# jafarinia/snuffy

Hardware: AMD Instinct MI355X
Metric: slides/sec (higher is better)
Workload: dtype f32; 1 GPU; cfgB: MILNet eval forward, 1 bag/step/rank, N=32768 patches D=768 h=6 Lambda=200 (K=200) depth=1 relu mlp x4; parallelism=bag-parallel x1, bags_resident_per_rank=8, launch=hip graph replay, rccl_ranks=0

## Files before the change

### include/snuffy_hip.h

```cpp
#ifndef SNUFFY_HIP_H
#define SNUFFY_HIP_H

#include <stddef.h>
#include <stdint.h>

#ifdef __cplusplus
extern "C" {
#endif

typedef void* snf_stream_t;

#define SNF_OK 0
#define SNF_EINVAL (-1)
#define SNF_ELAUNCH (-2)
#define SNF_EUNSUPPORTED (-3)
#define SNF_EWORKSPACE (-4)

#define SNF_ACT_RELU 0
#define SNF_ACT_GELU 1
#define SNF_ACT_LEAKYRELU 2
#define SNF_ACT_SELU 3
#define SNF_ACT_NONE 4

#define SNF_DT_F32 0
// ... 58 lines not shown
                     const void* gate_bf16, void* dst_bf16, float* partial, snf_stream_t stream);
int snf_dropout_rows_bf16(void* x, int64_t ldx, int64_t m, int n, float dropout_p, uint64_t seed, uint64_t offset, snf_stream_t stream);
int snf_residual_assemble_dropout_f32(const float* x, int64_t n, int d, const void* add_bf16, const float* add_bias,
                                      const int32_t* slot_map, const float* delta_rows, float dropout_p, uint64_t seed, uint64_t offset,
                                      float* z_out, snf_stream_t stream);
int snf_colsum_fused_dropout(const void* src, int src_dtype, int64_t n, int d, float dropout_p, uint64_t seed, uint64_t offset,
                             void* dst_bf16, float* partial, snf_stream_t stream);
int snf_split3_colsum_f32(const float* x, int64_t ldx, int64_t m, int k, const void* gate_bf16, int64_t ldg, void* out_bf16,
                          int64_t ldo, int64_t plane, float* partial, snf_stream_t stream);
int snf_split_hl_colsum_f32(const float* x, int64_t ldx, int64_t m, int k, const void* gate_hl, int64_t ldg, void* out_hl, int64_t ldo,
                            float* partial, snf_stream_t stream);
int snf_linear_rows_x3_f32(const float* x, int64_t ldx, const float* w, int64_t ldw, const float* bias, int r, int c, int k, void* out,
                           int64_t ldo, int out_dtype, snf_stream_t stream);
int snf_linear_rows_x3_resid_f32(const float* x, int64_t ldx, const float* w, int64_t ldw, const float* bias, const float* resid, int64_t ldr,
                                 int r, int c, int k, float* out, int64_t ldo, float* out2, int64_t ldo2, snf_stream_t stream);
int snf_critic_ln_hl_f32(const float* x, int64_t n, int d, const float* w, const float* b, int c_out, float* scores,
                         const float* gamma, const float* beta, float eps, void* out_hl, void* selector_state,
                         snf_stream_t stream);
int snf_layernorm_rows_split3_f32(const float* x, int64_t n, int d, const int32_t* slot_map, const float* patch_rows,
                                  const float* gamma, const float* beta, float eps, void* out_bf16, snf_stream_t stream);

int snf_bias_act(void* h, int dtype, int64_t n, int f, const float* bias, int act, snf_stream_t stream);

size_t snf_ln_mean_head_workspace_bytes(int d);
int snf_ln_mean_head_f32(const float* z, int64_t n, int d, const void* add_bf16, const float* add_bias,
                         const int32_t* slot_map, const float* delta_rows, float* z_out, const float* gamma,
                         const float* beta, float eps, const float* w_head, const float* b_head, int c_out,
                         float* logits, float* pooled, void* workspace, size_t workspace_bytes, snf_stream_t stream);
int snf_ln_mean_head_deferred_f32(const float* z, int64_t n, int d, const float* slabs, const int32_t* tile_map, int tiles_n,
                                  const void* add_bf16, const float* add_bias, const int32_t* slot_map, const float* delta_rows,
                                  float* z_out, const float* gamma, const float* beta, float eps, const float* w_head,
                                  const float* b_head, int c_out, float* logits, float* pooled, void* workspace,
                                  size_t workspace_bytes, snf_stream_t stream);

size_t snf_sparse_attn_fwd_workspace_bytes(int64_t n, int k, int h, int dk, int mfma);
int snf_sparse_attn_fwd_f32(const float* q, const float* kp, const float* v, int64_t n, int k, int h, int dk,
                            float scale, float* out, float* attn, float* lse, void* workspace,
                            size_t workspace_bytes, snf_stream_t stream);
int snf_sparse_attn_fwd_x3u_f32(const float* q, int64_t ldq, const float* kp, const float* v, int64_t ldv, int64_t n, int k, int h, int dk,
                                float scale, float* out, float* attn, float* lse, void* workspace, size_t workspace_bytes,
                                snf_stream_t stream);
int snf_sparse_attn_fwd_mfma(const void* q, int64_t ldq, const void* v, int64_t ldv, int qv_dtype, const void* kp,
                             int kp_dtype, int64_t n, int k, int h, int dk, float scale, float* out, float* attn,
                             float* lse, void* workspace, size_t workspace_bytes, snf_stream_t stream);

int snf_sparse_attn_fwd_mfma_dropout(const void* q, int64_t ldq, const void* v, int64_t ldv, int qv_dtype, const void* kp,
                                     int kp_dtype, int64_t n, int k, int h, int dk, float scale, float* out, float* attn,
                                     float* lse, float dropout_p, uint64_t seed, uint64_t offset, void* workspace,
                                     size_t workspace_bytes, snf_stream_t stream);
int snf_sparse_attn_bwd_mfma_dropout(const void* q, int64_t ldq, const void* v, int64_t ldv, int qv_dtype, const float* kp,
                                     const float* dout, const float* lse, const float* mask, float dropout_p, uint64_t seed,
                                     uint64_t offset, int64_t n, int k, int h, int dk, float scale, float* dq, float* dv,
                                     void* ds, int ds_dtype, snf_stream_t stream);
int snf_dropout_mask_f32(float dropout_p, uint64_t seed, uint64_t offset, int h, int64_t n, int k, float* mask,
                         snf_stream_t stream);

size_t snf_sparse_attn_fwd_x3_workspace_bytes(int64_t n, int k, int h, int dk);
int snf_sparse_attn_fwd_x3(const float* q, int64_t ldq, const float* v, int64_t ldv, const float* kp, int64_t n, int k, int h,
                           int dk, float scale, float* out, float* attn, float* lse, void* workspace, size_t workspace_bytes,
                           snf_stream_t stream);
int snf_sparse_attn_fwd_x3_dropout(const float* q, int64_t ldq, const float* v, int64_t ldv, const float* kp, int64_t n, int k, int h,
                                   int dk, float scale, float dropout_p, uint64_t seed, uint64_t offset, float* out, float* attn,
                                   float* lse, void* workspace, size_t workspace_bytes, snf_stream_t stream);

size_t snf_sparse_attn_fwd_x3_hl_workspace_bytes(int64_t n, int k, int h, int dk);
int snf_sparse_attn_fwd_x3_hl(const void* q_hl, int64_t ldq, const void* v_hl, int64_t ldv, const float* kp, int64_t n, int k, int h,
// ... 150 lines not shown
```

### snuffy_amd/_ffi.py

```python
import ctypes
import os
from ctypes import c_char_p, c_float, c_int, c_int64, c_size_t, c_uint64, c_void_p

_HERE = os.path.dirname(os.path.abspath(__file__))
LIB_PATH = os.environ.get("SNUFFY_HIP_LIB") or os.path.join(_HERE, "lib", "libsnuffy_hip.so")

SNF_OK = 0
SNF_EINVAL = -1
SNF_ELAUNCH = -2
SNF_EUNSUPPORTED = -3
SNF_EWORKSPACE = -4

ACT_CODES = {"relu": 0, "gelu": 1, "leakyrelu": 2, "selu": 3, "none": 4}
DT_F32 = 0
DT_BF16 = 1
DT_BF16_SPLIT3 = 2
DT_BF16_HL = 3
TOPK_MAX_K = 2048

SIGNATURES = {
    "snf_version": (c_char_p, []),
    "snf_last_error": (c_char_p, []),
    "snf_device_cu_count": (c_int, []),
    "snf_critic_f32": (c_int, [c_void_p, c_int64, c_int, c_void_p, c_void_p, c_int, c_void_p, c_void_p, c_void_p,
# ... 15 lines not shown
    "snf_slot_map_i32": (c_int, [c_void_p, c_int, c_int64, c_void_p, c_void_p]),
    "snf_gather_slot_map_f32": (c_int, [c_void_p, c_int64, c_int, c_void_p, c_int, c_void_p, c_void_p, c_void_p, c_void_p]),
    "snf_layernorm_rows_f32": (c_int, [c_void_p, c_int64, c_int, c_void_p, c_void_p, c_void_p, c_void_p, c_float,
                                       c_void_p, c_void_p, c_void_p, c_void_p, c_void_p, c_void_p]),
    "snf_layernorm_bwd_blocks": (c_int, [c_int64]),
    "snf_layernorm_rows_bwd_f32": (c_int, [c_void_p, c_int64, c_int, c_void_p, c_int, c_int64, c_void_p, c_float, c_void_p,
                                           c_void_p, c_void_p, c_void_p, c_void_p]),
    "snf_fold_blocks": (c_int, [c_int]),
    "snf_fold_linear_f32": (c_int, [c_void_p, c_int, c_int, c_void_p, c_void_p, c_void_p, c_void_p, c_int64, c_void_p, c_void_p,
                                    c_void_p]),
    "snf_unfold_linear_f32": (c_int, [c_void_p, c_void_p, c_int, c_int, c_void_p, c_void_p, c_void_p, c_void_p, c_void_p,
                                      c_void_p]),
    "snf_split3_f32": (c_int, [c_void_p, c_int64, c_int64, c_int, c_void_p, c_void_p]),
    "snf_mil_loss_f32": (c_int, [c_void_p, c_int64, c_int, c_void_p, c_void_p, c_void_p, c_void_p, c_void_p, c_void_p, c_void_p, c_void_p]),
    "snf_mil_loss_bwd_f32": (c_int, [c_void_p, c_void_p, c_void_p, c_int64, c_int, c_void_p, c_void_p, c_void_p]),
    "snf_split3_weight_f32": (c_int, [c_void_p, c_int64, c_int64, c_int, c_void_p, c_void_p, c_void_p]),
    "snf_split3_colsum_f32": (c_int, [c_void_p, c_int64, c_int64, c_int, c_void_p, c_int64, c_void_p, c_int64, c_int64, c_void_p, c_void_p]),
    "snf_colsum_blocks": (c_int, [c_int64]),
    "snf_colsum_fused": (c_int, [c_void_p, c_int, c_int64, c_int, c_void_p, c_int64, c_void_p, c_void_p, c_void_p, c_void_p]),
    "snf_layernorm_rows_split3_f32": (c_int, [c_void_p, c_int64, c_int, c_void_p, c_void_p, c_void_p, c_void_p, c_float,
                                              c_void_p, c_void_p]),
    "snf_linear_rows_x3_f32": (c_int, [c_void_p, c_int64, c_void_p, c_int64, c_void_p, c_int, c_int, c_int, c_void_p, c_int64, c_int,
                                       c_void_p]),
    "snf_critic_ln_hl_f32": (c_int, [c_void_p, c_int64, c_int, c_void_p, c_void_p, c_int, c_void_p, c_void_p, c_void_p, c_float,
                                     c_void_p, c_void_p, c_void_p]),
    "snf_bias_act": (c_int, [c_void_p, c_int, c_int64, c_int, c_void_p, c_int, c_void_p]),
    "snf_ln_mean_head_workspace_bytes": (c_size_t, [c_int]),
    "snf_ln_mean_head_f32": (c_int, [c_void_p, c_int64, c_int, c_void_p, c_void_p, c_void_p, c_void_p, c_void_p,
                                     c_void_p, c_void_p, c_float, c_void_p, c_void_p, c_int, c_void_p, c_void_p,
                                     c_void_p, c_size_t, c_void_p]),
    "snf_ln_mean_head_deferred_f32": (c_int, [c_void_p, c_int64, c_int, c_void_p, c_void_p, c_int, c_void_p, c_void_p, c_void_p, c_void_p,
                                              c_void_p, c_void_p, c_void_p, c_float, c_void_p, c_void_p, c_int, c_void_p, c_void_p,
                                              c_void_p, c_size_t, c_void_p]),
    "snf_sparse_attn_fwd_workspace_bytes": (c_size_t, [c_int64, c_int, c_int, c_int, c_int]),
    "snf_sparse_attn_fwd_f32": (c_int, [c_void_p, c_void_p, c_void_p, c_int64, c_int, c_int, c_int, c_float, c_void_p,
                                        c_void_p, c_void_p, c_void_p, c_size_t, c_void_p]),
    "snf_sparse_attn_fwd_x3u_f32": (c_int, [c_void_p, c_int64, c_void_p, c_void_p, c_int64, c_int64, c_int, c_int, c_int, c_float, c_void_p,
                                            c_void_p, c_void_p, c_void_p, c_size_t, c_void_p]),
    "snf_sparse_attn_bwd_workspace_bytes": (c_size_t, [c_int64, c_int, c_int, c_int]),
    "snf_sparse_attn_bwd_f32": (c_int, [c_void_p, c_void_p, c_void_p, c_void_p, c_void_p, c_void_p, c_int64, c_int, c_int,
                                        c_int, c_float, c_void_p, c_void_p, c_void_p, c_void_p, c_size_t, c_void_p]),
    "snf_sparse_attn_bwd_ld_f32": (c_int, [c_void_p, c_int64, c_void_p, c_void_p, c_int64, c_void_p, c_void_p, c_void_p, c_int64, c_int, c_int,
                                           c_int, c_float, c_void_p, c_void_p, c_void_p, c_void_p, c_size_t, c_void_p]),
    "snf_sparse_attn_bwd_dropout_f32": (c_int, [c_void_p, c_int64, c_void_p, c_void_p, c_int64, c_void_p, c_float, c_uint64, c_uint64, c_void_p,
                                                c_int64, c_int, c_int, c_int, c_float, c_void_p, c_void_p, c_void_p, c_void_p, c_size_t, c_void_p]),
    "snf_sparse_attn_bwd_mfma": (c_int, [c_void_p, c_int64, c_void_p, c_int64, c_int, c_void_p, c_void_p, c_void_p, c_void_p,
                                         c_int64, c_int, c_int, c_int, c_float, c_void_p, c_void_p, c_void_p, c_int, c_void_p]),
    "snf_sparse_attn_dkp_f32": (c_int, [c_void_p, c_void_p, c_int64, c_int, c_int, c_int, c_void_p, c_void_p, c_size_t,
                                        c_void_p]),
    "snf_sparse_attn_fwd_mfma": (c_int, [c_void_p, c_int64, c_void_p, c_int64, c_int, c_void_p, c_int, c_int64, c_int, c_int,
                                         c_int, c_float, c_void_p, c_void_p, c_void_p, c_void_p, c_size_t, c_void_p]),
    "snf_sparse_attn_fwd_x3_workspace_bytes": (c_size_t, [c_int64, c_int, c_int, c_int]),
    "snf_sparse_attn_fwd_x3": (c_int, [c_void_p, c_int64, c_void_p, c_int64, c_void_p, c_int64, c_int, c_int, c_int, c_float,
                                       c_void_p, c_void_p, c_void_p, c_void_p, c_size_t, c_void_p]),
    "snf_sparse_attn_fwd_x3_dropout": (c_int, [c_void_p, c_int64, c_void_p, c_int64, c_void_p, c_int64, c_int, c_int, c_int, c_float,
                                               c_float, c_uint64, c_uint64, c_void_p, c_void_p, c_void_p, c_void_p, c_size_t, c_void_p]),
    "snf_sparse_attn_fwd_x3_hl_workspace_bytes": (c_size_t, [c_int64, c_int, c_int, c_int]),
    "snf_sparse_attn_x3_hl_kpfrag_bytes": (c_size_t, [c_int, c_int, c_int]),
    "snf_linear_rows_x3_kpfrag_f32": (c_int, [c_void_p, c_int64, c_void_p, c_int64, c_void_p, c_int, c_int, c_int, c_int, c_float,
                                              c_void_p, c_size_t, c_void_p]),
    "snf_gather_linear_rows_x3_kpfrag_f32": (c_int, [c_void_p, c_int64, c_int64, c_void_p, c_void_p, c_int64, c_void_p, c_int, c_int, c_int,
                                                     c_int, c_float, c_void_p, c_size_t, c_void_p, c_void_p, c_void_p]),
    "snf_sparse_attn_fwd_x3_hl_kpfrag": (c_int, [c_void_p, c_int64, c_void_p, c_int64, c_void_p, c_int64, c_int, c_int, c_int,
                                                 c_void_p, c_void_p, c_void_p, c_void_p, c_size_t, c_void_p]),
    "snf_sparse_attn_fwd_x3_hl": (c_int, [c_void_p, c_int64, c_void_p, c_int64, c_void_p, c_int64, c_int, c_int, c_int, c_float,
                                          c_void_p, c_void_p, c_void_p, c_void_p, c_size_t, c_void_p]),
# ... 133 lines not shown
```

### snuffy_amd/csrc/rowops.hip

```cpp
#include <math.h>

#include "common.h"
#include "philox.h"
#include "selector.h"

namespace {

constexpr int WG = 256;
constexpr int WAVES = WG / 64;

template <int VEC>
struct VecT;
template <>
struct VecT<4> {
    using type = float4;
};
template <>
struct VecT<1> {
    using type = float;
};

template <int VEC, int NV>
struct RowRegs {
    float v[NV * VEC];
// ... 1017 lines not shown
                    hi += bias[col + 2 * t + 1];
                }
                w[t] = pack_bf16x2(apply_act(lo, act), apply_act(hi, act));
            }
            *reinterpret_cast<uint4*>(h + i8) = make_uint4(w[0], w[1], w[2], w[3]);
        }
    } else {
        for (int64_t i = (int64_t)blockIdx.x * blockDim.x + threadIdx.x; i < total; i += (int64_t)gridDim.x * blockDim.x) {
            float v = bf16_bits_to_f32(h[i]) + (bias ? bias[i % f] : 0.f);
            h[i] = f32_to_bf16_bits(apply_act(v, act));
        }
    }
}

template <int VEC, int NV>
__device__ __forceinline__ void add_row_bf16(const unsigned short* __restrict__ row, int d, int lane, float (&r)[NV * VEC]) {
#pragma unroll
    for (int i = 0; i < NV; ++i) {
        int e = (i * 64 + lane) * VEC;
        if (e < d) {
            if constexpr (VEC == 4) {
                uint2 p = *reinterpret_cast<const uint2*>(row + e);
                r[i * 4 + 0] += __uint_as_float(p.x << 16);
                r[i * 4 + 1] += __uint_as_float(p.x & 0xffff0000u);
                r[i * 4 + 2] += __uint_as_float(p.y << 16);
                r[i * 4 + 3] += __uint_as_float(p.y & 0xffff0000u);
            } else {
                r[i] += bf16_bits_to_f32(row[e]);
            }
        }
    }
}

template <int VEC, int NV, bool DEFER = false>
__global__ __launch_bounds__(WG) void ln_colsum_kernel(const float* __restrict__ z, int64_t n, int d, float eps,
                                                       const unsigned short* __restrict__ add_bf16,
                                                       const float* __restrict__ add_bias,
                                                       const int32_t* __restrict__ slot_map,
                                                       const float* __restrict__ delta_rows,
                                                       float* __restrict__ z_out,
                                                       float* __restrict__ partial ,
                                                       const int* __restrict__ vl = nullptr, int vl_bags = 0,
                                                       const float* __restrict__ slabs = nullptr,
                                                       const int32_t* __restrict__ tile_map = nullptr, int tiles_n = 0) {
    const int lane = threadIdx.x & 63;
    const int wave = threadIdx.x >> 6;
    int bid = blockIdx.x, gdim = gridDim.x;
    if (vl) {
        const int* __restrict__ dsc = vl + 4 * vl[4 * vl_bags + bid];
        const int64_t row0 = dsc[1];
        bid -= dsc[0];
        n = dsc[2];
        gdim = dsc[3];
        z += row0 * d;
        if (add_bf16) add_bf16 += row0 * d;
        if (slot_map) slot_map += row0;
        if (z_out) z_out += row0 * d;
    }
    float acc[NV * VEC];
#pragma unroll
    for (int i = 0; i < NV * VEC; ++i) acc[i] = 0.f;
    float bias_r[NV * VEC];
    if (add_bias) load_row<VEC, NV>(add_bias, d, lane, bias_r);
    const float inv_d = 1.0f / (float)d;
    const int64_t rstride = (int64_t)gdim * WAVES;
    float nz[NV * VEC];
    uint2 nb[NV];
    constexpr int NCB = DEFER ? (NV * VEC * 64 + 255) / 256 : 1;
    float ns[DEFER ? NV * VEC : 1];
    int mp_n[NCB], mp_nn[NCB];
    auto lookup = [&](int64_t row, int (&mp)[NCB]) __attribute__((always_inline)) {
        const int trow = __builtin_amdgcn_readfirstlane((int)(row >> 8));
#pragma unroll
        for (int cb = 0; cb < NCB; ++cb) mp[cb] = cb < tiles_n ? tile_map[(int64_t)trow * tiles_n + cb] : 0;
    };
    auto issue = [&](int64_t row) __attribute__((always_inline)) {
        load_row<VEC, NV>(z + row * d, d, lane, nz);
// ... 75 lines not shown
            int sl = slot_map[row];
            if (sl >= 0) {
                float dr[NV * VEC];
                load_row<VEC, NV>(delta_rows + (int64_t)sl * d, d, lane, dr);
#pragma unroll
                for (int i = 0; i < NV * VEC; ++i) r[i] += dr[i];
            }
        }
        if (z_out) store_row_f32<VEC, NV>(z_out + row * d, d, lane, r);
        float s1 = 0.f;
#pragma unroll
        for (int i = 0; i < NV * VEC; ++i) s1 += r[i];
        const float mean = wave_sum(s1) * inv_d;
        float s2 = 0.f;
#pragma unroll
        for (int i = 0; i < NV; ++i) {
#pragma unroll
            for (int t = 0; t < VEC; ++t) {
                int e = (i * 64 + lane) * VEC + t;
                float dv = (e < d) ? (r[i * VEC + t] - mean) : 0.f;
                s2 = fmaf(dv, dv, s2);
            }
        }
        const float rstd = 1.0f / sqrtf(wave_sum(s2) * inv_d + eps);
#pragma unroll
        for (int i = 0; i < NV * VEC; ++i) acc[i] += (r[i] - mean) * rstd;
    }
    extern __shared__ float lds[];
    float* mine = lds + wave * (NV * VEC * 64);
#pragma unroll
    for (int i = 0; i < NV * VEC; ++i) mine[i * 64 + lane] = acc[i];
    __syncthreads();
    if (wave == 0) {
#pragma unroll
        for (int i = 0; i < NV; ++i) {
#pragma unroll
            for (int t = 0; t < VEC; ++t) {
                float s = 0.f;
                for (int w2 = 0; w2 < WAVES; ++w2) s += lds[w2 * (NV * VEC * 64) + (i * VEC + t) * 64 + lane];
                int e = (i * 64 + lane) * VEC + t;
                if (e < d) partial[(int64_t)blockIdx.x * d + e] = s;
            }
        }
    }
}

constexpr int HEAD_NSLICE = 16;
__global__ __launch_bounds__(256) void ln_colreduce_kernel(const float* __restrict__ partial, int nparts, int d,
                                                           float* __restrict__ partial2 ,
                                                           const int* __restrict__ vl = nullptr) {
    __shared__ float red[4][64];
    if (vl) {
        const int* __restrict__ dsc = vl + 4 * blockIdx.z;
        partial += (int64_t)dsc[0] * d;
        nparts = dsc[3];
        partial2 += (int64_t)blockIdx.z * HEAD_NSLICE * d;
    }
    const int c = threadIdx.x & 63, wv = threadIdx.x >> 6;
    const int e = blockIdx.x * 64 + c;
    const int sl = blockIdx.y;
    float s = 0.f;
    if (e < d)
        for (int p = sl + HEAD_NSLICE * wv; p < nparts; p += HEAD_NSLICE * 4) s += partial[(int64_t)p * d + e];
    red[wv][c] = s;
    __syncthreads();
    if (wv == 0 && e < d) partial2[(int64_t)sl * d + e] = ((red[0][c] + red[1][c]) + red[2][c]) + red[3][c];
}

__global__ __launch_bounds__(256) void head_gemv_kernel(const float* __restrict__ partial2, int64_t n, int d,
                                                        const float* __restrict__ gamma, const float* __restrict__ beta,
                                                        const float* __restrict__ w_head, const float* __restrict__ b_head,
                                                        float* __restrict__ pooled_out, float* __restrict__ logits,
                                                        const int* __restrict__ vl = nullptr) {
    __shared__ float red[256];
    if (vl) {
        partial2 += (int64_t)blockIdx.y * HEAD_NSLICE * d;
        n = vl[4 * blockIdx.y + 2];
        logits += (int64_t)blockIdx.y * gridDim.x;
        if (pooled_out) pooled_out += (int64_t)blockIdx.y * d;
    }
// ... 670 lines not shown
                "snf_gather_slot_map_f32: bad shape n=%lld d=%d k=%d (k <= 2048)", (long long)n, d, k);
    const int64_t grid = k + (n + WG - 1) / WG;
    hipLaunchKernelGGL(gather_slot_map_kernel, dim3((unsigned)grid), dim3(WG), 0, snf::as_stream(stream), x, n, d, idx, k, xs,
                       map, reinterpret_cast<__bf16*>(xs_bf16));
    return snf::check_launch("gather_slot_map_kernel");
}

int snf_bias_act(void* h, int dtype, int64_t n, int f, const float* bias, int act, snf_stream_t stream) {
    SNF_REQUIRE(h, "snf_bias_act: null h");
    SNF_REQUIRE(n >= 1 && f >= 1, "snf_bias_act: bad shape");
    SNF_REQUIRE(act >= SNF_ACT_RELU && act <= SNF_ACT_NONE, "snf_bias_act: unknown activation %d", act);
    SNF_REQUIRE(dtype == SNF_DT_F32 || dtype == SNF_DT_BF16, "snf_bias_act: unknown dtype %d", dtype);
    SNF_REQUIRE(aligned16(h) && (!bias || aligned16(bias)), "snf_bias_act: buffers must be 16-byte aligned");
    const int64_t total = n * (int64_t)f;
    const int per = dtype == SNF_DT_F32 ? 4 : 8;
    int64_t want = (total / per + WG - 1) / WG;
    int64_t cap = (int64_t)snf::cu_count() * 8;
    int grid = (int)(want < cap ? (want > 0 ? want : 1) : cap);
    hipStream_t s = snf::as_stream(stream);
    if (dtype == SNF_DT_F32)
        hipLaunchKernelGGL(bias_act_f32_kernel, dim3(grid), dim3(WG), 0, s, reinterpret_cast<float*>(h), n, f, bias, act);
    else
        hipLaunchKernelGGL(bias_act_bf16_kernel, dim3(grid), dim3(WG), 0, s, reinterpret_cast<unsigned short*>(h), n, f,
                           bias, act);
    return snf::check_launch("bias_act_kernel");
}

static int ln_head_parts(int64_t n) {
    int64_t want = (n + WAVES - 1) / WAVES;
    int64_t cap = (int64_t)snf::cu_count() * 4;
    return (int)(want < cap ? (want > 0 ? want : 1) : cap);
}

size_t snf_ln_mean_head_workspace_bytes(int d) {
    if (d < 1) return 0;
    return ((size_t)snf::cu_count() * 4 + HEAD_NSLICE) * (size_t)d * sizeof(float);
}

static int ln_mean_head_impl(const float* z, int64_t n, int d, const float* slabs, const int32_t* tile_map, int tiles_n,
                             const void* add_bf16, const float* add_bias, const int32_t* slot_map, const float* delta_rows,
                             float* z_out, const float* gamma, const float* beta, float eps, const float* w_head,
                             const float* b_head, int c_out, float* logits, float* pooled, void* workspace, size_t workspace_bytes,
                             snf_stream_t stream) {
    SNF_REQUIRE(z && w_head && logits && workspace, "snf_ln_mean_head_f32: null pointer");
    SNF_REQUIRE(!slot_map || delta_rows, "snf_ln_mean_head_f32: slot_map without delta_rows");
    SNF_REQUIRE(n >= 1 && d >= 1 && c_out >= 1, "snf_ln_mean_head_f32: bad shape");
    const int parts = ln_head_parts(n);
    if (workspace_bytes < ((size_t)parts + HEAD_NSLICE) * d * sizeof(float)) {
        snf::set_error("snf_ln_mean_head_f32: workspace %zu < %zu", workspace_bytes,
                       ((size_t)parts + HEAD_NSLICE) * d * sizeof(float));
        return SNF_EWORKSPACE;
    }
    RowCfg cfg;
    const bool al = aligned16(z) && (!add_bf16 || aligned16(add_bf16)) && (!add_bias || aligned16(add_bias)) &&
                    (!delta_rows || aligned16(delta_rows)) && (!z_out || aligned16(z_out));
    SNF_REQUIRE(pick_row_cfg(d, al, &cfg), "snf_ln_mean_head_f32: d=%d too wide (max 2048)", d);
    hipStream_t s = snf::as_stream(stream);
    float* partial = reinterpret_cast<float*>(workspace);
    float* partial2 = partial + (size_t)parts * d;
    if (tile_map) {
        SNF_ROW_DISPATCH(cfg, hipLaunchKernelGGL((ln_colsum_kernel<VEC, NV, true>), dim3(parts), dim3(WG),
                                                  WAVES * NV * VEC * 64 * sizeof(float), s, z, n, d, eps,
                                                  reinterpret_cast<const unsigned short*>(add_bf16), add_bias, slot_map,
                                                  delta_rows, z_out, partial, nullptr, 0, slabs, tile_map, tiles_n));
    } else {
        SNF_ROW_DISPATCH(cfg, hipLaunchKernelGGL((ln_colsum_kernel<VEC, NV>), dim3(parts), dim3(WG),
                                                  WAVES * NV * VEC * 64 * sizeof(float), s, z, n, d, eps,
                                                  reinterpret_cast<const unsigned short*>(add_bf16), add_bias, slot_map,
                                                  delta_rows, z_out, partial));
    }
    int rc = snf::check_launch("ln_colsum_kernel");
    if (rc) return rc;
    hipLaunchKernelGGL(ln_colreduce_kernel, dim3((d + 63) / 64, HEAD_NSLICE), dim3(256), 0, s, partial, parts, d, partial2);
    rc = snf::check_launch("ln_colreduce_kernel");
    if (rc) return rc;
    hipLaunchKernelGGL(head_gemv_kernel, dim3(c_out), dim3(256), 0, s, partial2, n, d, gamma, beta, w_head, b_head, pooled,
                       logits);
    return snf::check_launch("head_gemv_kernel");
}

int snf_ln_mean_head_f32(const float* z, int64_t n, int d, const void* add_bf16, const float* add_bias,
                         const int32_t* slot_map, const float* delta_rows, float* z_out, const float* gamma,
                         const float* beta, float eps, const float* w_head, const float* b_head, int c_out, float* logits,
                         float* pooled, void* workspace, size_t workspace_bytes, snf_stream_t stream) {
    return ln_mean_head_impl(z, n, d, nullptr, nullptr, 0, add_bf16, add_bias, slot_map, delta_rows, z_out, gamma, beta, eps, w_head,
                             b_head, c_out, logits, pooled, workspace, workspace_bytes, stream);
}

int snf_ln_mean_head_deferred_f32(const float* z, int64_t n, int d, const float* slabs, const int32_t* tile_map, int tiles_n,
                                  const void* add_bf16, const float* add_bias, const int32_t* slot_map, const float* delta_rows,
                                  float* z_out, const float* gamma, const float* beta, float eps, const float* w_head,
                                  const float* b_head, int c_out, float* logits, float* pooled, void* workspace,
                                  size_t workspace_bytes, snf_stream_t stream) {
    SNF_REQUIRE(slabs && tile_map, "snf_ln_mean_head_deferred_f32: null slabs / tile map");
    SNF_REQUIRE(aligned16(slabs) && tiles_n >= 1 && d <= 256 * (int64_t)tiles_n,
                "snf_ln_mean_head_deferred_f32: d=%d beyond %d column tiles (or unaligned slabs)", d, tiles_n);
    return ln_mean_head_impl(z, n, d, slabs, tile_map, tiles_n, add_bf16, add_bias, slot_map, delta_rows, z_out, gamma, beta, eps,
                             w_head, b_head, c_out, logits, pooled, workspace, workspace_bytes, stream);
}

int snf_ln_mean_head_varlen_plan(const int64_t* offsets, int bags, int d, int32_t* table, size_t table_ints,
                                 size_t* table_ints_needed, size_t* workspace_bytes) {
    SNF_REQUIRE(offsets && bags >= 1 && d >= 1, "snf_ln_mean_head_varlen_plan: bad arguments");
    int64_t total = 0;
    for (int b = 0; b < bags; ++b) {
        const int64_t n = offsets[b + 1] - offsets[b];
        SNF_REQUIRE(n >= 1 && offsets[b + 1] < 0x7fffffffll, "snf_ln_mean_head_varlen_plan: bag %d has %lld rows", b, (long long)n);
        total += ln_head_parts(n);
    }
    SNF_REQUIRE(total < 0x3fffffff, "snf_ln_mean_head_varlen_plan: too many workgroups");
    const size_t need = (size_t)4 * bags + (size_t)total;
    if (table_ints_needed) *table_ints_needed = need;
    if (workspace_bytes) *workspace_bytes = ((size_t)total + (size_t)bags * HEAD_NSLICE) * d * sizeof(float);
    if (table) {
        SNF_REQUIRE(table_ints >= need, "snf_ln_mean_head_varlen_plan: table %zu < %zu ints", table_ints, need);
        int64_t wg = 0;
        for (int b = 0; b < bags; ++b) {
            const int64_t n = offsets[b + 1] - offsets[b];
            const int parts = ln_head_parts(n);
            table[4 * b + 0] = (int32_t)wg, table[4 * b + 1] = (int32_t)offsets[b], table[4 * b + 2] = (int32_t)n;
            table[4 * b + 3] = parts;
            for (int i = 0; i < parts; ++i) table[(size_t)4 * bags + wg + i] = b;
            wg += parts;
        }
    }
    return SNF_OK;
}

int snf_ln_mean_head_varlen_f32(const float* z, const int64_t* offsets, int bags, int d, const void* add_bf16,
                                const float* add_bias, const int32_t* slot_map, const float* delta_rows, float* z_out,
                                const float* gamma, const float* beta, float eps, const float* w_head, const float* b_head,
// ... 69 lines not shown
```

### snuffy_amd/ops.py

```python
import ctypes
import math

import torch

from . import _ffi
from ._ffi import ACT_CODES, DT_BF16, DT_BF16_HL, DT_BF16_SPLIT3, DT_F32, TOPK_MAX_K, check


def _p(t):
    return None if t is None else ctypes.c_void_p(t.data_ptr())


_raw_stream = getattr(torch._C, "_cuda_getCurrentRawStream", None)


def _stream():
    if _raw_stream is not None:
        return ctypes.c_void_p(_raw_stream(torch.cuda.current_device()))
    return ctypes.c_void_p(torch.cuda.current_stream().cuda_stream)


def _on_current_device(t, name):
    if t.device.index != torch.cuda.current_device():
        raise _ffi.SnuffyHipError("%s lives on %s but the current device is cuda:%d: select the tensor's device first "
# ... 373 lines not shown
    check(_ffi.load().snf_fold_linear_f32(_p(w), r, c, _p(gamma), _p(beta), _p(bias), _p(out_w), out_w.stride(0), _p(out_bf),
                                          _p(out_bf16), _stream()), "snf_fold_linear_f32")


def unfold_linear(dwf, w, gamma, beta, dbf):
    dwf = _req(dwf, torch.float32, "dwf", 2)
    w = _req(w, torch.float32, "w", 2)
    r, c = w.shape
    gamma = _req(gamma, torch.float32, "gamma", 1)
    beta = _req(beta, torch.float32, "beta", 1)
    dbf = _req(dbf, torch.float32, "dbf", 1)
    lib = _ffi.load()
    dw = torch.empty(r, c, dtype=torch.float32, device=w.device)
    part = torch.empty(lib.snf_fold_blocks(r), 2, c, dtype=torch.float32, device=w.device)
    check(lib.snf_unfold_linear_f32(_p(dwf), _p(w), r, c, _p(gamma), _p(beta), _p(dbf), _p(dw), _p(part), _stream()),
          "snf_unfold_linear_f32")
    sums = part.sum(0)
    return dw, sums[0], sums[1]


def bias_act_(h, bias, act):
    if not h.is_cuda or not h.is_contiguous() or h.dim() != 2:
        raise _ffi.SnuffyHipError("bias_act_: h must be a contiguous 2-D GPU tensor")
    dt = {torch.float32: DT_F32, torch.bfloat16: DT_BF16}.get(h.dtype)
    if dt is None:
        raise TypeError("bias_act_: h must be float32 or bfloat16")
    if bias is not None:
        bias = _req(bias, torch.float32, "bias", 1)
    check(_ffi.load().snf_bias_act(_p(h), dt, h.shape[0], h.shape[1], _p(bias), ACT_CODES[act], _stream()),
          "snf_bias_act")
    return h


def ln_mean_head(z, gamma, beta, eps, w_head, b_head, add_bf16=None, add_bias=None, slot=None, delta_rows=None,
                 want_z=False, deferred=None):
    z = _req(z, torch.float32, "z", 2)
    n, d = z.shape
    if add_bf16 is not None:
        add_bf16 = _req(add_bf16, torch.bfloat16, "add_bf16", 2)
    if add_bias is not None:
        add_bias = _req(add_bias, torch.float32, "add_bias", 1)
    if slot is not None:
        slot = _req(slot, torch.int32, "slot", 1)
        delta_rows = _req(delta_rows, torch.float32, "delta_rows", 2)
    z_out = torch.empty_like(z) if want_z else None
    gamma = _req(gamma, torch.float32, "gamma", 1)
    beta = _req(beta, torch.float32, "beta", 1)
    w_head = _req(w_head, torch.float32, "w_head", 2)
    if b_head is not None:
        b_head = _req(b_head, torch.float32, "b_head", 1)
    c = w_head.shape[0]
    lib = _ffi.load()
    logits = torch.empty(c, dtype=torch.float32, device=z.device)
    pooled = torch.empty(d, dtype=torch.float32, device=z.device)
    wsb = lib.snf_ln_mean_head_workspace_bytes(d)
    ws = _ws(wsb, z.device)
    if deferred is not None:
        if tuple(deferred.tile_map.shape) != ((n + 255) // 256, (d + 255) // 256):
            raise ValueError("ln_mean_head: deferred part of a %s-tile result with z %s" % (tuple(deferred.tile_map.shape), (n, d)))
        check(lib.snf_ln_mean_head_deferred_f32(_p(z), n, d, _p(deferred.slabs), _p(deferred.tile_map), deferred.tile_map.shape[1],
                                                _p(add_bf16), _p(add_bias), _p(slot), _p(delta_rows), _p(z_out), _p(gamma), _p(beta),
                                                float(eps), _p(w_head), _p(b_head), c, _p(logits), _p(pooled), _p(ws), wsb, _stream()),
              "snf_ln_mean_head_deferred_f32")
        return logits, pooled, z_out
    check(lib.snf_ln_mean_head_f32(_p(z), n, d, _p(add_bf16), _p(add_bias), _p(slot), _p(delta_rows), _p(z_out),
                                   _p(gamma), _p(beta), float(eps), _p(w_head), _p(b_head), c, _p(logits), _p(pooled),
                                   _p(ws), wsb, _stream()), "snf_ln_mean_head_f32")
    return logits, pooled, z_out


def attn_bwd_dropout_supported(k, dk):
    return 1 <= k <= 1024 and k % 4 == 0 and dk % 8 == 0


def sparse_attn_bwd(q, kp, v, p, dout, h, mask=None, scale=None, dropout=None):
    if q.dtype != torch.float32 or v.dtype != torch.float32:
        raise TypeError("sparse_attn_bwd: q and v must be float32")
    kp = _req(kp, torch.float32, "kp", 2)
    if q.dim() == 2 and kp.dim() == 2 and (q.shape[1] // h) % 8 == 0 and kp.shape[0] <= 1024:
        q, v = _rows16(q, "q"), _rows16(v, "v")
    else:
        q, v = _req(q, torch.float32, "q", 2), _req(v, torch.float32, "v", 2)
    p = _req(p, torch.float32, "p", 3)
    dout = _req(dout, torch.float32, "dout", 2)
    if mask is not None:
        mask = _req(mask, torch.float32, "mask", 3)
    n, d = q.shape
    k = kp.shape[0]
    dk = d // h
    if p.shape != (h, n, k) or dout.shape != (k, d) or (mask is not None and mask.shape != p.shape):
        raise ValueError("sparse_attn_bwd: inconsistent shapes")
    scale = 1.0 / math.sqrt(dk) if scale is None else scale
    lib = _ffi.load()
    dq = torch.empty(n, d, dtype=torch.float32, device=q.device)
    dv = torch.empty(n, d, dtype=torch.float32, device=q.device)
    dkp = torch.empty_like(kp)
    wsb = lib.snf_sparse_attn_bwd_workspace_bytes(n, k, h, dk)
    ws = _ws(wsb, q.device)
    if dropout is not None and mask is None and float(dropout[0]) > 0.0:
        check(lib.snf_sparse_attn_bwd_dropout_f32(_p(q), q.stride(0), _p(kp), _p(v), v.stride(0), _p(p), float(dropout[0]),
# ... 1265 lines not shown
```

### snuffy_amd/snuffy.py

```python
import copy
import math

import numpy as np
import torch
import torch.nn as nn

from . import functional as SF
from . import ops

device = torch.device("cuda" if torch.cuda.is_available() else "cpu")


class RuntimeConfig:

    def __init__(self, precision="fp32", return_attention=True):
        self.stack = None
        self.sampler = "reference"
        self._device_sampler = None
        self._draws = 0
        self.set(precision, return_attention)

    def set_sampler(self, sampler):
        if sampler not in ("reference", "device"):
            raise ValueError("sampler must be 'reference' or 'device', got %r" % (sampler,))
# ... 237 lines not shown
        return self

    def forward(self, x):
        if self._graph_ok(x):
            return self._forward_graph(x)
        return self._forward_eager(x)

    def _forward_eager(self, x):
        for layer in self.b_classifier.encoder.layers[:1]:
            layer._xhat_offer = None
            layer._xn3_offer = None
        feats, classes = self._critic(x)
        prediction_bag, A = self.b_classifier(feats, classes)
        return classes, prediction_bag, A

    _GRAPH_SHAPES = 1024
    _GRAPH_COPY_BYTES = 32 << 20

    def _graph_ok(self, x):
        lim = getattr(self, "_graph_max_patches", 0)
        if lim <= 0 or self.training or torch.is_grad_enabled():
            return False
        if not (isinstance(x, torch.Tensor) and x.is_cuda and x.dim() == 3 and x.shape[0] == 1 and x.dtype == torch.float32
                and x.is_contiguous() and 0 < x.shape[1] <= lim and type(self.i_classifier) is FCLayer):
            return False
        if self.b_classifier.cfg.return_attention and x.numel() * 4 > self._GRAPH_COPY_BYTES:
            return False
        on_device = self.b_classifier.cfg.sampler == "device"
        return all(type(l) is EncoderLayer and (l.random_patch_share == 0 or on_device) for l in self.b_classifier.encoder.layers)

    def _weights_signature(self):
        plist = list(self.parameters())
        knobs = tuple((l.big_lambda, l.random_patch_share) for l in self.b_classifier.encoder.layers)
        knobs += (SF.FP32_GEMM, SF.FP32_ATTENTION, SF.X3_HL_ATTENTION, SF.X3_HL_KPFRAG, SF.X3_HL_KPFRAG_GATHER, SF.FP32_SHARED_NORM, ops.GEMM_HL_SPLITK, ops.GEMM_HL_DEFERRED,
                  SF.BF16_DEEP_STACKS, self.b_classifier.cfg.sampler)
        return tuple(SF.param_key(p) for p in plist), knobs

    def invalidate(self):
        if getattr(self, "_graph_max_patches", 0):
            self._graphs.clear()
            self._graph_seen.clear()
            self._graph_sig = None
        for layer in self.b_classifier.encoder.layers:
            SF.invalidate_folded(layer)
        SF.drop_param_caches(self)
        return self

    _GRAPH_STATE = ("_graphs", "_graph_seen", "_graph_pool", "_graph_sig", "_packed_bags", "_capture_stream")

    def __deepcopy__(self, memo):
        new = self.__class__.__new__(self.__class__)
        memo[id(self)] = new
        for k, v in self.__dict__.items():
            if k not in self._GRAPH_STATE:
                new.__dict__[k] = copy.deepcopy(v, memo)
        if getattr(self, "_graph_max_patches", 0):
            new._graphs, new._graph_seen, new._graph_pool = {}, set(), None
        new.b_classifier.cfg._device_sampler = None
        return new

    def _forward_graph(self, x):
        sig = self._weights_signature()
        if sig != getattr(self, "_graph_sig", None):
            self._graphs.clear()
            self._graph_seen.clear()
            self._graph_sig = sig
        cfg = self.b_classifier.cfg
# ... 94 lines not shown
```

Before: 930.8 slides/s.

## Fuse LN column reduction and head into colsum kernel via last-arriver tickets

Folds the second-stage column reduction and the pooled LayerNorm-mean head into the tail of ln_colsum_kernel. Atomic tickets per slice pick the last-arriving block, which finishes the reduction and computes logits, so the separate reduce and head kernel launches go away. Each call now needs a memset of the ticket words, and the final work runs serialized in a single block. It also adds a debug environment lookup on the host path, but that is absorbed under graph replay.

```diff
diff --git a/include/snuffy_hip.h b/include/snuffy_hip.h
--- a/include/snuffy_hip.h
+++ b/include/snuffy_hip.h
@@ -114,6 +114,15 @@
                                   float* z_out, const float* gamma, const float* beta, float eps, const float* w_head,
                                   const float* b_head, int c_out, float* logits, float* pooled, void* workspace,
                                   size_t workspace_bytes, snf_stream_t stream);
+int snf_ln_mean_head_fused_f32(const float* z, int64_t n, int d, const void* add_bf16, const float* add_bias,
+                               const int32_t* slot_map, const float* delta_rows, float* z_out, const float* gamma,
+                               const float* beta, float eps, const float* w_head, const float* b_head, int c_out,
+                               float* logits, float* pooled, void* workspace, size_t workspace_bytes, snf_stream_t stream);
+int snf_ln_mean_head_deferred_fused_f32(const float* z, int64_t n, int d, const float* slabs, const int32_t* tile_map, int tiles_n,
+                                        const void* add_bf16, const float* add_bias, const int32_t* slot_map, const float* delta_rows,
+                                        float* z_out, const float* gamma, const float* beta, float eps, const float* w_head,
+                                        const float* b_head, int c_out, float* logits, float* pooled, void* workspace,
+                                        size_t workspace_bytes, snf_stream_t stream);
 
 size_t snf_sparse_attn_fwd_workspace_bytes(int64_t n, int k, int h, int dk, int mfma);
 int snf_sparse_attn_fwd_f32(const float* q, const float* kp, const float* v, int64_t n, int k, int h, int dk,
diff --git a/snuffy_amd/_ffi.py b/snuffy_amd/_ffi.py
--- a/snuffy_amd/_ffi.py
+++ b/snuffy_amd/_ffi.py
@@ -71,6 +71,12 @@
     "snf_ln_mean_head_deferred_f32": (c_int, [c_void_p, c_int64, c_int, c_void_p, c_void_p, c_int, c_void_p, c_void_p, c_void_p, c_void_p,
                                               c_void_p, c_void_p, c_void_p, c_float, c_void_p, c_void_p, c_int, c_void_p, c_void_p,
                                               c_void_p, c_size_t, c_void_p]),
+    "snf_ln_mean_head_fused_f32": (c_int, [c_void_p, c_int64, c_int, c_void_p, c_void_p, c_void_p, c_void_p, c_void_p,
+                                           c_void_p, c_void_p, c_float, c_void_p, c_void_p, c_int, c_void_p, c_void_p,
+                                           c_void_p, c_size_t, c_void_p]),
+    "snf_ln_mean_head_deferred_fused_f32": (c_int, [c_void_p, c_int64, c_int, c_void_p, c_void_p, c_int, c_void_p, c_void_p, c_void_p,
+                                                    c_void_p, c_void_p, c_void_p, c_void_p, c_float, c_void_p, c_void_p, c_int, c_void_p,
+                                                    c_void_p, c_void_p, c_size_t, c_void_p]),
     "snf_sparse_attn_fwd_workspace_bytes": (c_size_t, [c_int64, c_int, c_int, c_int, c_int]),
     "snf_sparse_attn_fwd_f32": (c_int, [c_void_p, c_void_p, c_void_p, c_int64, c_int, c_int, c_int, c_float, c_void_p,
                                         c_void_p, c_void_p, c_void_p, c_size_t, c_void_p]),
diff --git a/snuffy_amd/csrc/rowops.hip b/snuffy_amd/csrc/rowops.hip
--- a/snuffy_amd/csrc/rowops.hip
+++ b/snuffy_amd/csrc/rowops.hip
@@ -1073,7 +1073,113 @@
     }
 }
 
-template <int VEC, int NV, bool DEFER = false>
+constexpr int HEAD_NSLICE = 16;
+struct HeadTail {
+    float* partial2 = nullptr;
+    unsigned int* tickets = nullptr;
+    const float* gamma = nullptr;
+    const float* beta = nullptr;
+    const float* w_head = nullptr;
+    const float* b_head = nullptr;
+    float* pooled = nullptr;
+    float* logits = nullptr;
+    int c_out = 0;
+};
+
+template <int VEC, int NV>
+__device__ __forceinline__ void store_row_sc1(float* row, int d, int lane, const float (&r)[NV * VEC]) {
+    typedef unsigned int u32x4 __attribute__((ext_vector_type(4)));
+    const __amdgpu_buffer_rsrc_t rs = __builtin_amdgcn_make_buffer_rsrc(row, 0, d * (int)sizeof(float), 0x00020000);
+#pragma unroll
+    for (int i = 0; i < NV; ++i) {
+        const int e = (i * 64 + lane) * VEC;
+        if (e < d) {
+            if constexpr (VEC == 4) {
+                const u32x4 v = {__float_as_uint(r[i * 4]), __float_as_uint(r[i * 4 + 1]), __float_as_uint(r[i * 4 + 2]),
+                                 __float_as_uint(r[i * 4 + 3])};
+                __builtin_amdgcn_raw_buffer_store_b128(v, rs, e * (int)sizeof(float), 0,  16);
+            } else {
+                __builtin_amdgcn_raw_buffer_store_b32(__float_as_uint(r[i]), rs, e * (int)sizeof(float), 0,  16);
+            }
+        }
+    }
+}
+
+__device__ __forceinline__ bool head_last_arriver(unsigned int* ticket, unsigned target, volatile unsigned int* word) {
+    asm volatile("s_waitcnt vmcnt(0)" ::: "memory");
+    __syncthreads();
+    if (threadIdx.x == 0) *word = __hip_atomic_fetch_add(ticket, 1u, __ATOMIC_RELAXED, __HIP_MEMORY_SCOPE_AGENT);
+    __syncthreads();
+    const bool last = *word == target - 1u;
+    __syncthreads();
+    if (!last) return false;
+    if (threadIdx.x == 0) {
+        __builtin_amdgcn_fence(__ATOMIC_ACQUIRE, "agent");
+        asm volatile("s_waitcnt vmcnt(0)" ::: "memory");
+        __hip_atomic_store(ticket, 0u, __ATOMIC_RELAXED, __HIP_MEMORY_SCOPE_AGENT);
+    }
+    __syncthreads();
+    return true;
+}
+
+template <int VEC, int NV>
+__device__ void ln_head_tail(const float* partial, int parts, int64_t n, int d, const HeadTail& T, float* lds ) {
+    const int lane = threadIdx.x & 63;
+    const int wave = threadIdx.x >> 6;
+    const int sl = blockIdx.x % HEAD_NSLICE;
+    volatile unsigned int* word = reinterpret_cast<volatile unsigned int*>(lds);
+    if (!T.tickets) return;
+    if (!head_last_arriver(T.tickets + sl, (unsigned)((parts - sl + HEAD_NSLICE - 1) / HEAD_NSLICE), word)) return;
+    if (!T.partial2) return;
+    {
+        float s[NV * VEC];
+#pragma unroll
+        for (int i = 0; i < NV * VEC; ++i) s[i] = 0.f;
+#pragma unroll 4
+        for (int p = sl + HEAD_NSLICE * wave; p < parts; p += HEAD_NSLICE * WAVES) {
+            float r[NV * VEC];
+            load_row<VEC, NV>(partial + (int64_t)p * d, d, lane, r);
+#pragma unroll
+            for (int i = 0; i < NV * VEC; ++i) s[i] += r[i];
+        }
+        float* mine = lds + wave * (NV * VEC * 64);
+#pragma unroll
+        for (int i = 0; i < NV * VEC; ++i) mine[i * 64 + lane] = s[i];
+        __syncthreads();
+        if (wave == 0) {
+            float v[NV * VEC];
+#pragma unroll
+            for (int i = 0; i < NV * VEC; ++i) {
+                const float* q = lds + i * 64 + lane;
+                v[i] = ((q[0] + q[NV * VEC * 64]) + q[2 * NV * VEC * 64]) + q[3 * NV * VEC * 64];
+            }
+            store_row_sc1<VEC, NV>(T.partial2 + (int64_t)sl * d, d, lane, v);
+        }
+    }
+    if (!head_last_arriver(T.tickets + HEAD_NSLICE, (unsigned)(parts < HEAD_NSLICE ? parts : HEAD_NSLICE), word)) return;
+    const float inv_n = 1.0f / (float)n;
+    for (int c = 0; c < T.c_out; ++c) {
+        float acc = 0.f;
+        for (int e = threadIdx.x; e < d; e += 256) {
+            float t = 0.f;
+#pragma unroll
+            for (int s2 = 0; s2 < HEAD_NSLICE; ++s2) t += s2 < parts ? T.partial2[(int64_t)s2 * d + e] : 0.f;
+            const float v = (T.gamma ? T.gamma[e] : 1.f) * (t * inv_n) + (T.beta ? T.beta[e] : 0.f);
+            if (c == 0 && T.pooled) T.pooled[e] = v;
+            acc = fmaf(T.w_head[(int64_t)c * d + e], v, acc);
+        }
+        __syncthreads();
+        lds[threadIdx.x] = acc;
+        __syncthreads();
+        for (int s2 = 128; s2 > 0; s2 >>= 1) {
+            if ((int)threadIdx.x < s2) lds[threadIdx.x] += lds[threadIdx.x + s2];
+            __syncthreads();
+        }
+        if (threadIdx.x == 0) T.logits[c] = lds[0] + (T.b_head ? T.b_head[c] : 0.f);
+    }
+}
+
+template <int VEC, int NV, bool DEFER = false, bool FUSE = false>
 __global__ __launch_bounds__(WG) void ln_colsum_kernel(const float* __restrict__ z, int64_t n, int d, float eps,
                                                        const unsigned short* __restrict__ add_bf16,
                                                        const float* __restrict__ add_bias,
@@ -1083,7 +1189,8 @@
                                                        float* __restrict__ partial ,
                                                        const int* __restrict__ vl = nullptr, int vl_bags = 0,
                                                        const float* __restrict__ slabs = nullptr,
-                                                       const int32_t* __restrict__ tile_map = nullptr, int tiles_n = 0) {
+                                                       const int32_t* __restrict__ tile_map = nullptr, int tiles_n = 0,
+                                                       HeadTail tail = HeadTail{}) {
     const int lane = threadIdx.x & 63;
     const int wave = threadIdx.x >> 6;
     int bid = blockIdx.x, gdim = gridDim.x;
@@ -1225,6 +1332,7 @@
     for (int i = 0; i < NV * VEC; ++i) mine[i * 64 + lane] = acc[i];
     __syncthreads();
     if (wave == 0) {
+        float ps[FUSE ? NV * VEC : 1];
 #pragma unroll
         for (int i = 0; i < NV; ++i) {
 #pragma unroll
@@ -1232,13 +1340,19 @@
                 float s = 0.f;
                 for (int w2 = 0; w2 < WAVES; ++w2) s += lds[w2 * (NV * VEC * 64) + (i * VEC + t) * 64 + lane];
                 int e = (i * 64 + lane) * VEC + t;
-                if (e < d) partial[(int64_t)blockIdx.x * d + e] = s;
-            }
-        }
-    }
-}
-
-constexpr int HEAD_NSLICE = 16;
+                if constexpr (FUSE) {
+                    ps[i * VEC + t] = s;
+                } else {
+                    if (e < d) partial[(int64_t)blockIdx.x * d + e] = s;
+                }
+            }
+        }
+        if constexpr (FUSE) store_row_sc1<VEC, NV>(partial + (int64_t)blockIdx.x * d, d, lane, ps);
+    }
+    if constexpr (FUSE) ln_head_tail<VEC, NV>(partial, (int)gridDim.x, n, d, tail, lds);
+}
+
+__global__ void head_zero_kernel(unsigned int* t) { if (threadIdx.x < 32) t[threadIdx.x] = 0u; }
 __global__ __launch_bounds__(256) void ln_colreduce_kernel(const float* __restrict__ partial, int nparts, int d,
                                                            float* __restrict__ partial2 ,
                                                            const int* __restrict__ vl = nullptr) {
@@ -1975,23 +2089,26 @@
     return (int)(want < cap ? (want > 0 ? want : 1) : cap);
 }
 
+constexpr size_t HEAD_TICKET_BYTES = 128;
+static_assert(HEAD_TICKET_BYTES >= (HEAD_NSLICE + 1) * sizeof(unsigned int), "ticket block");
+
 size_t snf_ln_mean_head_workspace_bytes(int d) {
     if (d < 1) return 0;
-    return ((size_t)snf::cu_count() * 4 + HEAD_NSLICE) * (size_t)d * sizeof(float);
+    return ((size_t)snf::cu_count() * 4 + HEAD_NSLICE) * (size_t)d * sizeof(float) + HEAD_TICKET_BYTES;
 }
 
 static int ln_mean_head_impl(const float* z, int64_t n, int d, const float* slabs, const int32_t* tile_map, int tiles_n,
                              const void* add_bf16, const float* add_bias, const int32_t* slot_map, const float* delta_rows,
                              float* z_out, const float* gamma, const float* beta, float eps, const float* w_head,
                              const float* b_head, int c_out, float* logits, float* pooled, void* workspace, size_t workspace_bytes,
-                             snf_stream_t stream) {
+                             snf_stream_t stream, bool fuse = false) {
     SNF_REQUIRE(z && w_head && logits && workspace, "snf_ln_mean_head_f32: null pointer");
     SNF_REQUIRE(!slot_map || delta_rows, "snf_ln_mean_head_f32: slot_map without delta_rows");
     SNF_REQUIRE(n >= 1 && d >= 1 && c_out >= 1, "snf_ln_mean_head_f32: bad shape");
     const int parts = ln_head_parts(n);
-    if (workspace_bytes < ((size_t)parts + HEAD_NSLICE) * d * sizeof(float)) {
-        snf::set_error("snf_ln_mean_head_f32: workspace %zu < %zu", workspace_bytes,
-                       ((size_t)parts + HEAD_NSLICE) * d * sizeof(float));
+    const size_t need = ((size_t)parts + HEAD_NSLICE) * d * sizeof(float) + (fuse ? HEAD_TICKET_BYTES : 0);
+    if (workspace_bytes < need) {
+        snf::set_error("snf_ln_mean_head_f32: workspace %zu < %zu", workspace_bytes, need);
         return SNF_EWORKSPACE;
     }
     RowCfg cfg;
@@ -1999,8 +2116,32 @@
                     (!delta_rows || aligned16(delta_rows)) && (!z_out || aligned16(z_out));
     SNF_REQUIRE(pick_row_cfg(d, al, &cfg), "snf_ln_mean_head_f32: d=%d too wide (max 2048)", d);
     hipStream_t s = snf::as_stream(stream);
-    float* partial = reinterpret_cast<float*>(workspace);
+    float* partial = reinterpret_cast<float*>(reinterpret_cast<unsigned char*>(workspace) + (fuse ? HEAD_TICKET_BYTES : 0));
     float* partial2 = partial + (size_t)parts * d;
+    if (fuse) {
+        SNF_REQUIRE(cfg.vec == 1 || aligned16(workspace), "snf_ln_mean_head_fused_f32: the workspace must be 16-byte aligned");
+        HeadTail T;
+        T.partial2 = partial2;
+        T.tickets = reinterpret_cast<unsigned int*>(workspace);
+        T.gamma = gamma, T.beta = beta, T.w_head = w_head, T.b_head = b_head, T.pooled = pooled, T.logits = logits, T.c_out = c_out;
+        const int dbg = getenv("SNF_HEAD_DBG") ? atoi(getenv("SNF_HEAD_DBG")) : 0;
+        if (dbg & 1) hipLaunchKernelGGL(head_zero_kernel, dim3(1), dim3(64), 0, s, T.tickets);
+        else if (hipMemsetAsync(T.tickets, 0, HEAD_TICKET_BYTES, s) != hipSuccess) return snf::check_launch("hipMemsetAsync");
+        if (dbg & 2) T.partial2 = nullptr;
+        if (dbg & 4) T.tickets = nullptr;
+        if (tile_map) {
+            SNF_ROW_DISPATCH(cfg, hipLaunchKernelGGL((ln_colsum_kernel<VEC, NV, true, true>), dim3(parts), dim3(WG),
+                                                      WAVES * NV * VEC * 64 * sizeof(float), s, z, n, d, eps,
+                                                      reinterpret_cast<const unsigned short*>(add_bf16), add_bias, slot_map,
+                                                      delta_rows, z_out, partial, nullptr, 0, slabs, tile_map, tiles_n, T));
+        } else {
+            SNF_ROW_DISPATCH(cfg, hipLaunchKernelGGL((ln_colsum_kernel<VEC, NV, false, true>), dim3(parts), dim3(WG),
+                                                      WAVES * NV * VEC * 64 * sizeof(float), s, z, n, d, eps,
+                                                      reinterpret_cast<const unsigned short*>(add_bf16), add_bias, slot_map,
+                                                      delta_rows, z_out, partial, nullptr, 0, nullptr, nullptr, 0, T));
+        }
+        return snf::check_launch("ln_colsum_kernel<fused head>");
+    }
     if (tile_map) {
         SNF_ROW_DISPATCH(cfg, hipLaunchKernelGGL((ln_colsum_kernel<VEC, NV, true>), dim3(parts), dim3(WG),
                                                   WAVES * NV * VEC * 64 * sizeof(float), s, z, n, d, eps,
@@ -2030,16 +2171,42 @@
                              b_head, c_out, logits, pooled, workspace, workspace_bytes, stream);
 }
 
+int snf_ln_mean_head_fused_f32(const float* z, int64_t n, int d, const void* add_bf16, const float* add_bias,
+                               const int32_t* slot_map, const float* delta_rows, float* z_out, const float* gamma,
+                               const float* beta, float eps, const float* w_head, const float* b_head, int c_out, float* logits,
+                               float* pooled, void* workspace, size_t workspace_bytes, snf_stream_t stream) {
+    return ln_mean_head_impl(z, n, d, nullptr, nullptr, 0, add_bf16, add_bias, slot_map, delta_rows, z_out, gamma, beta, eps, w_head,
+                             b_head, c_out, logits, pooled, workspace, workspace_bytes, stream, true);
+}
+
+static int ln_mean_head_deferred_impl(const float* z, int64_t n, int d, const float* slabs, const int32_t* tile_map, int tiles_n,
+                                      const void* add_bf16, const float* add_bias, const int32_t* slot_map, const float* delta_rows,
+                                      float* z_out, const float* gamma, const float* beta, float eps, const float* w_head,
+                                      const float* b_head, int c_out, float* logits, float* pooled, void* workspace,
+                                      size_t workspace_bytes, snf_stream_t stream, bool fuse) {
+    SNF_REQUIRE(slabs && tile_map, "snf_ln_mean_head_deferred_f32: null slabs / tile map");
+    SNF_REQUIRE(aligned16(slabs) && tiles_n >= 1 && d <= 256 * (int64_t)tiles_n,
+                "snf_ln_mean_head_deferred_f32: d=%d beyond %d column tiles (or unaligned slabs)", d, tiles_n);
+    return ln_mean_head_impl(z, n, d, slabs, tile_map, tiles_n, add_bf16, add_bias, slot_map, delta_rows, z_out, gamma, beta, eps,
+                             w_head, b_head, c_out, logits, pooled, workspace, workspace_bytes, stream, fuse);
+}
+
 int snf_ln_mean_head_deferred_f32(const float* z, int64_t n, int d, const float* slabs, const int32_t* tile_map, int tiles_n,
                                   const void* add_bf16, const float* add_bias, const int32_t* slot_map, const float* delta_rows,
                                   float* z_out, const float* gamma, const float* beta, float eps, const float* w_head,
                                   const float* b_head, int c_out, float* logits, float* pooled, void* workspace,
                                   size_t workspace_bytes, snf_stream_t stream) {
-    SNF_REQUIRE(slabs && tile_map, "snf_ln_mean_head_deferred_f32: null slabs / tile map");
-    SNF_REQUIRE(aligned16(slabs) && tiles_n >= 1 && d <= 256 * (int64_t)tiles_n,
-                "snf_ln_mean_head_deferred_f32: d=%d beyond %d column tiles (or unaligned slabs)", d, tiles_n);
-    return ln_mean_head_impl(z, n, d, slabs, tile_map, tiles_n, add_bf16, add_bias, slot_map, delta_rows, z_out, gamma, beta, eps,
-                             w_head, b_head, c_out, logits, pooled, workspace, workspace_bytes, stream);
+    return ln_mean_head_deferred_impl(z, n, d, slabs, tile_map, tiles_n, add_bf16, add_bias, slot_map, delta_rows, z_out, gamma, beta,
+                                      eps, w_head, b_head, c_out, logits, pooled, workspace, workspace_bytes, stream, false);
+}
+
+int snf_ln_mean_head_deferred_fused_f32(const float* z, int64_t n, int d, const float* slabs, const int32_t* tile_map, int tiles_n,
+                                        const void* add_bf16, const float* add_bias, const int32_t* slot_map, const float* delta_rows,
+                                        float* z_out, const float* gamma, const float* beta, float eps, const float* w_head,
+                                        const float* b_head, int c_out, float* logits, float* pooled, void* workspace,
+                                        size_t workspace_bytes, snf_stream_t stream) {
+    return ln_mean_head_deferred_impl(z, n, d, slabs, tile_map, tiles_n, add_bf16, add_bias, slot_map, delta_rows, z_out, gamma, beta,
+                                      eps, w_head, b_head, c_out, logits, pooled, workspace, workspace_bytes, stream, true);
 }
 
 int snf_ln_mean_head_varlen_plan(const int64_t* offsets, int bags, int d, int32_t* table, size_t table_ints,
diff --git a/snuffy_amd/ops.py b/snuffy_amd/ops.py
--- a/snuffy_amd/ops.py
+++ b/snuffy_amd/ops.py
@@ -429,6 +429,9 @@
     return h
 
 
+LN_HEAD_FUSED = True
+
+
 def ln_mean_head(z, gamma, beta, eps, w_head, b_head, add_bf16=None, add_bias=None, slot=None, delta_rows=None,
                  want_z=False, deferred=None):
     z = _req(z, torch.float32, "z", 2)
@@ -455,14 +458,16 @@
     if deferred is not None:
         if tuple(deferred.tile_map.shape) != ((n + 255) // 256, (d + 255) // 256):
             raise ValueError("ln_mean_head: deferred part of a %s-tile result with z %s" % (tuple(deferred.tile_map.shape), (n, d)))
-        check(lib.snf_ln_mean_head_deferred_f32(_p(z), n, d, _p(deferred.slabs), _p(deferred.tile_map), deferred.tile_map.shape[1],
-                                                _p(add_bf16), _p(add_bias), _p(slot), _p(delta_rows), _p(z_out), _p(gamma), _p(beta),
-                                                float(eps), _p(w_head), _p(b_head), c, _p(logits), _p(pooled), _p(ws), wsb, _stream()),
+        fn = lib.snf_ln_mean_head_deferred_fused_f32 if LN_HEAD_FUSED else lib.snf_ln_mean_head_deferred_f32
+        check(fn(_p(z), n, d, _p(deferred.slabs), _p(deferred.tile_map), deferred.tile_map.shape[1],
+                 _p(add_bf16), _p(add_bias), _p(slot), _p(delta_rows), _p(z_out), _p(gamma), _p(beta),
+                 float(eps), _p(w_head), _p(b_head), c, _p(logits), _p(pooled), _p(ws), wsb, _stream()),
               "snf_ln_mean_head_deferred_f32")
         return logits, pooled, z_out
-    check(lib.snf_ln_mean_head_f32(_p(z), n, d, _p(add_bf16), _p(add_bias), _p(slot), _p(delta_rows), _p(z_out),
-                                   _p(gamma), _p(beta), float(eps), _p(w_head), _p(b_head), c, _p(logits), _p(pooled),
-                                   _p(ws), wsb, _stream()), "snf_ln_mean_head_f32")
+    fn = lib.snf_ln_mean_head_fused_f32 if LN_HEAD_FUSED else lib.snf_ln_mean_head_f32
+    check(fn(_p(z), n, d, _p(add_bf16), _p(add_bias), _p(slot), _p(delta_rows), _p(z_out),
+             _p(gamma), _p(beta), float(eps), _p(w_head), _p(b_head), c, _p(logits), _p(pooled),
+             _p(ws), wsb, _stream()), "snf_ln_mean_head_f32")
     return logits, pooled, z_out
 
 
diff --git a/snuffy_amd/snuffy.py b/snuffy_amd/snuffy.py
--- a/snuffy_amd/snuffy.py
+++ b/snuffy_amd/snuffy.py
@@ -293,7 +293,7 @@
     def _weights_signature(self):
         plist = list(self.parameters())
         knobs = tuple((l.big_lambda, l.random_patch_share) for l in self.b_classifier.encoder.layers)
-        knobs += (SF.FP32_GEMM, SF.FP32_ATTENTION, SF.X3_HL_ATTENTION, SF.X3_HL_KPFRAG, SF.X3_HL_KPFRAG_GATHER, SF.FP32_SHARED_NORM, ops.GEMM_HL_SPLITK, ops.GEMM_HL_DEFERRED,
+        knobs += (SF.FP32_GEMM, SF.FP32_ATTENTION, SF.X3_HL_ATTENTION, SF.X3_HL_KPFRAG, SF.X3_HL_KPFRAG_GATHER, SF.FP32_SHARED_NORM, ops.GEMM_HL_SPLITK, ops.GEMM_HL_DEFERRED, ops.LN_HEAD_FUSED,
                   SF.BF16_DEEP_STACKS, self.b_classifier.cfg.sampler)
         return tuple(SF.param_key(p) for p in plist), knobs
 
```

Measured after the change: 929.4 slides/s. Within noise of the previous version (-0.1%).
